# RS2002/PianoBart

Hardware: AMD Instinct MI355X
Metric: Octuple tokens/sec/GPU (seq=1024, 12L/768d) pretrain step; %MFMA peak (higher is better)
Workload: dtype bf16

## Files before the change

### pianobart_amd/csrc/pb_fa_tiles.h

```cpp
#pragma once
#include "pb_common.h"
#include "pb_api_internal.h"

namespace {


constexpr int HD = 64, FT = 256;
constexpr float LOG2E = 1.4426950408889634f;
typedef __attribute__((ext_vector_type(4))) short s16x4;
typedef __attribute__((ext_vector_type(8))) short s16x8;

struct Fa64Args {
    const bf16_t *q, *k, *v, *o, *dout;
    bf16_t *out, *dq, *dk, *dv;
    float* lse; const float* delta; const float* key_mask; const int* kmax;
    int B, H, Sq, Sk;
    long q_sb, q_ss, k_sb, k_ss, v_sb, v_ss, o_sb, o_ss, dq_sb, dq_ss, dk_sb, dk_ss, dv_sb, dv_ss;
    float scale; int causal;
    float* cs_q; float* cs_kv;
    const bf16_t* zeros;
    const int *vl_q_off, *vl_k_off, *vl_q_len, *vl_k_len;
    const int* bh_order;
};

inline Fa64Args fa64_args(const pb_attn_desc& d, bool bwd) {
    Fa64Args a = {};
    a.q = (const bf16_t*)d.q; a.k = (const bf16_t*)d.k; a.v = (const bf16_t*)d.v; a.dout = (const bf16_t*)d.dout;
    if (bwd) a.o = (const bf16_t*)d.o; else a.out = (bf16_t*)d.o;
    a.dq = (bf16_t*)d.dq; a.dk = (bf16_t*)d.dk; a.dv = (bf16_t*)d.dv; a.lse = d.lse; a.delta = d.delta;
    a.key_mask = d.key_mask; a.kmax = d.q_off ? d.k_vis : d.kmax;
    a.B = d.B; a.H = d.H; a.Sq = d.Sq; a.Sk = d.Sk;
    a.q_sb = d.q_sb; a.q_ss = d.q_ss; a.k_sb = d.k_sb; a.k_ss = d.k_ss; a.v_sb = d.v_sb; a.v_ss = d.v_ss; a.o_sb = d.o_sb; a.o_ss = d.o_ss;
    a.dq_sb = d.dq_sb; a.dq_ss = d.dq_ss; a.dk_sb = d.dk_sb; a.dk_ss = d.dk_ss; a.dv_sb = d.dv_sb; a.dv_ss = d.dv_ss;
    a.scale = d.scale; a.causal = d.flags & PB_ATTN_CAUSAL;
    a.zeros = (const bf16_t*)pb_zero_page();
    a.vl_q_off = d.q_off; a.vl_k_off = d.k_off; a.vl_q_len = d.q_len; a.vl_k_len = d.k_len; a.bh_order = d.bh_order;
    return a;
}

__device__ __forceinline__ void varlen_localize(Fa64Args& p, int b) {
    if (!p.vl_q_off) return;
    const long qo = p.vl_q_off[b], ko = p.vl_k_off[b];
    p.Sq = p.vl_q_len[b]; p.Sk = p.vl_k_len[b];
    p.q += qo * p.q_ss - b * p.q_sb; p.k += ko * p.k_ss - b * p.k_sb; p.v += ko * p.v_ss - b * p.v_sb;
    if (p.o) p.o += qo * p.o_ss - b * p.o_sb;
    if (p.out) p.out += qo * p.o_ss - b * p.o_sb;
    if (p.dout) p.dout += qo * p.o_ss - b * p.o_sb;
    if (p.dq) p.dq += qo * p.dq_ss - b * p.dq_sb;
    if (p.dk) p.dk += ko * p.dk_ss - b * p.dk_sb;
    if (p.dv) p.dv += ko * p.dv_ss - b * p.dv_sb;
}

#define MFMA16(a, b, c) __builtin_amdgcn_mfma_f32_16x16x32_bf16((a), (b), (c), 0, 0, 0)

__device__ __forceinline__ int fsw(int row) { return (((row >> 1) & 3) << 1) | ((row >> 3) & 1); }

__device__ __forceinline__ void glds16(const bf16_t* g, char* lds_wave_base) {
    __builtin_amdgcn_global_load_lds((const __attribute__((address_space(1))) void*)g,
                                     (__attribute__((address_space(3))) void*)lds_wave_base, 16, 0, 0);
}
struct StageOff { unsigned off[2]; unsigned chunk[2]; };
__device__ __forceinline__ StageOff stage_off(long ld, int wave, int lane) {
    StageOff o;
#pragma unroll
    for (int n = 0; n < 2; ++n) {
        const int row = (wave * 2 + n) * 8 + (lane >> 3);
        o.chunk[n] = (unsigned)((lane & 7) ^ fsw(row));
        o.off[n] = (unsigned)(row * ld + (o.chunk[n] << 3));
    }
    return o;
}
__device__ __forceinline__ void stage64(const bf16_t* __restrict__ base, long ld, int r0, int nrows, char* lds, int wave, int lane, const StageOff& so,
                                        int cmax = 8, const bf16_t* zeros = nullptr) {
    if (r0 + 64 <= nrows) {
        const bf16_t* tb = base + (long)r0 * ld;
#pragma unroll
        for (int n = 0; n < 2; ++n) glds16((cmax == 8 || (int)so.chunk[n] < cmax) ? tb + so.off[n] : zeros, lds + (wave * 2 + n) * 1024);
    } else {
#pragma unroll
        for (int n = 0; n < 2; ++n) {
            const int inst = wave * 2 + n;
            const int row = inst * 8 + (lane >> 3);
            const int chunk = (lane & 7) ^ fsw(row);
            const int gr = min(r0 + row, nrows - 1);
            glds16((cmax == 8 || chunk < cmax) ? base + (long)gr * ld + chunk * 8 : zeros, lds + inst * 1024);
        }
    }
}
__device__ __forceinline__ bf16x8 frag_row(const char* lds, int row, int ks, int g) {
    return *reinterpret_cast<const bf16x8*>(lds + row * 128 + (((ks * 4 + g) ^ fsw(row)) << 4));
}
__device__ __forceinline__ bf16x8 frag_tr(const char* lds, int c0, int s, int lane) {
    const int lr = lane & 15, g = lane >> 4, qq = lr >> 2, pp = lr & 3;
    const int chunk = (c0 >> 3) + (pp >> 1);
    const int r0 = 32 * s + 4 * g + qq, r1 = r0 + 16;
    const int o0 = r0 * 128 + ((chunk ^ fsw(r0)) << 4) + ((pp & 1) << 3);
    const int o1 = r1 * 128 + ((chunk ^ fsw(r1)) << 4) + ((pp & 1) << 3);
    const s16x4 lo = __builtin_amdgcn_ds_read_tr16_b64_v4i16((__attribute__((address_space(3))) s16x4*)(lds + o0));
    const s16x4 hi = __builtin_amdgcn_ds_read_tr16_b64_v4i16((__attribute__((address_space(3))) s16x4*)(lds + o1));
    const s16x8 v = {lo[0], lo[1], lo[2], lo[3], hi[0], hi[1], hi[2], hi[3]};
    return __builtin_bit_cast(bf16x8, v);
}
__device__ __forceinline__ bf16x8 pack_pair(const f32x4& lo, const f32x4& hi) {
    bf16x8 r = {(bf16_t)lo[0], (bf16_t)lo[1], (bf16_t)lo[2], (bf16_t)lo[3], (bf16_t)hi[0], (bf16_t)hi[1], (bf16_t)hi[2], (bf16_t)hi[3]};
    return r;
}
__device__ __forceinline__ bf16x8 frag_global(const bf16_t* __restrict__ g, long ld, int row, int nvalid, int col) {
    bf16x8 z = {};
    if (row < nvalid) z = *reinterpret_cast<const bf16x8*>(g + (long)row * ld + col);
    return z;
}
__device__ __forceinline__ float grp_max(float v) {
    auto a = __builtin_amdgcn_permlane16_swap(__float_as_uint(v), __float_as_uint(v), false, false);
    v = fmaxf(__uint_as_float(a[0]), __uint_as_float(a[1]));
    auto b = __builtin_amdgcn_permlane32_swap(__float_as_uint(v), __float_as_uint(v), false, false);
    return fmaxf(__uint_as_float(b[0]), __uint_as_float(b[1]));
}
__device__ __forceinline__ float grp_sum(float v) {
    auto a = __builtin_amdgcn_permlane16_swap(__float_as_uint(v), __float_as_uint(v), false, false);
    v = __uint_as_float(a[0]) + __uint_as_float(a[1]);
    auto b = __builtin_amdgcn_permlane32_swap(__float_as_uint(v), __float_as_uint(v), false, false);
    return __uint_as_float(b[0]) + __uint_as_float(b[1]);
}
template <bool V> struct BoolTag { static constexpr bool value = V; };

constexpr int STG = 2 * 8192 + 512;

__device__ __forceinline__ void block_map(int nrb, int H, int B, int& rb, int& h, int& b, const int* order = nullptr) {
    const int L = blockIdx.x, BH = H * B;
    int bh;
    if ((BH & 7) == 0) { const int x = L & 7, slot = L >> 3, j = slot / nrb; bh = j * 8 + x; rb = (slot - j * nrb + j) % nrb; }
    else { bh = L / nrb; rb = (L - bh * nrb + bh) % nrb; }
    if (order) bh = order[bh];
    h = bh % H; b = bh / H;
}

template <int OFF>
__device__ __forceinline__ void ds_tr(s16x4& d, unsigned addr) {
    asm volatile("ds_read_b64_tr_b16 %0, %1 offset:%2" : "=v"(d) : "v"(addr), "i"(OFF));
}
__device__ __forceinline__ unsigned tr_lane_off64(int c0, int lane) {
    const int lr = lane & 15, g = lane >> 4, qq = lr >> 2, pp = lr & 3;
    const int r0 = 4 * g + qq, chunk = (c0 >> 3) + (pp >> 1);
    return (unsigned)(r0 * 128 + ((chunk ^ fsw(r0)) << 4) + ((pp & 1) << 3));
}
__device__ __forceinline__ void ds_tr_block(s16x4 (&d)[2][2], unsigned addr) {
    ds_tr<0>(d[0][0], addr); ds_tr<2048>(d[0][1], addr); ds_tr<4096>(d[1][0], addr); ds_tr<6144>(d[1][1], addr);
}
__device__ __forceinline__ bf16x8 tr_join(s16x4 lo, s16x4 hi) {
    const s16x8 v = {lo[0], lo[1], lo[2], lo[3], hi[0], hi[1], hi[2], hi[3]};
    return __builtin_bit_cast(bf16x8, v);
}
#define TRW4(X) "+v"(X[0][0]), "+v"(X[0][1]), "+v"(X[1][0]), "+v"(X[1][1])
__device__ __forceinline__ void tr_wait4(s16x4 (&t)[4][2][2]) {
    asm volatile("s_waitcnt lgkmcnt(0)" : TRW4(t[0]), TRW4(t[1]), TRW4(t[2]), TRW4(t[3]));
}
__device__ __forceinline__ void tr_wait8(s16x4 (&t)[4][2][2], s16x4 (&u)[4][2][2]) {
    asm volatile("s_waitcnt lgkmcnt(0)" : TRW4(t[0]), TRW4(t[1]), TRW4(t[2]), TRW4(t[3]), TRW4(u[0]), TRW4(u[1]), TRW4(u[2]), TRW4(u[3]));
}
#undef TRW4
__device__ __forceinline__ unsigned lds_u32(const void* p) { return (unsigned)(uintptr_t)(__attribute__((address_space(3))) const char*)p; }

template <int N> __device__ __forceinline__ void wait_vm() { asm volatile("s_waitcnt vmcnt(%0)" :: "i"(N) : "memory"); }

template <int NB> struct FaCfg {
    static constexpr int NS = NB == 1 ? 3 : 2;
    static constexpr int STB = 2 * NB * 8192;
    static constexpr int PCS = 4 * NB;
    static constexpr int KT = NB == 1 ? 2 : 1;
};

__device__ __forceinline__ bf16x8 scale_frag(bf16x8 v, float c) {
    bf16x8 r;
#pragma unroll
    for (int e = 0; e < 8; ++e) r[e] = (bf16_t)((float)v[e] * c);
    return r;
}

}
```

### pianobart_amd/csrc/pb_flash64.hip

```cpp
#include "pb_common.h"
#include "pb_fa_tiles.h"

namespace {


constexpr float LAZY_THR = 8.0f;
template <int HD>
__global__ __launch_bounds__(FT) void fa64_fwd_kernel(const Fa64Args pin) {
    constexpr int NB = (HD + 63) / 64, KS = HD / 32, DT = HD / 16, HDT = HD;
    using C = FaCfg<NB>;
    extern __shared__ __attribute__((aligned(16))) char smem[];
    const int t = threadIdx.x, lane = t & 63, lr = lane & 15, g = lane >> 4;
    const int wave = __builtin_amdgcn_readfirstlane(t >> 6);
    int rb, h, b;
    block_map((pin.Sq + 127) / 128, pin.H, pin.B, rb, h, b, pin.bh_order);
    if (pin.causal) rb = (pin.Sq + 127) / 128 - 1 - rb;
    const int q0 = rb * 128;
    Fa64Args p = pin;
    varlen_localize(p, b);
    const int lse_ld = pin.Sq;
    if (q0 >= p.Sq) return;
    const bf16_t* Q = p.q + b * p.q_sb + h * HDT;
    const bf16_t* K = p.k + b * p.k_sb + h * HDT;
    const bf16_t* V = p.v + b * p.v_sb + h * HDT;
    const float c = p.scale * LOG2E;
    const int kvis_end = p.kmax ? min(p.Sk, p.kmax[b]) : p.Sk;
    const int kend = p.causal ? min(kvis_end, q0 + 128) : kvis_end;
    const int nt = (kend + 63) / 64;
    float* ldsBias = reinterpret_cast<float*>(smem + C::NS * C::STB);
    unsigned* ldsFlag = reinterpret_cast<unsigned*>(ldsBias + ((p.Sk + 63) / 64) * 64);
    for (int tile = wave; tile < nt; tile += 4) {
        const int key = tile * 64 + lane;
        const bool vis = key < (pin.vl_q_off ? kvis_end : p.Sk) && (!p.key_mask || p.key_mask[(long)b * p.Sk + key] != 0.f);
        ldsBias[key] = vis ? 0.f : -INFINITY;
        const bool allvis = __builtin_amdgcn_ballot_w64(vis) == ~0ull;
        if (lane == 0) ldsFlag[tile] = allvis ? 0u : 1u;
    }
    int myq[2];
    bf16x8 qf[2][KS];
#pragma unroll
    for (int qt = 0; qt < 2; ++qt) {
        myq[qt] = q0 + wave * 32 + qt * 16 + lr;
#pragma unroll
        for (int ks = 0; ks < KS; ++ks) qf[qt][ks] = scale_frag(frag_global(Q, p.q_ss, myq[qt], p.Sq, ks * 32 + g * 8), c);
    }
#pragma unroll
    for (int ks = 0; ks < KS; ++ks) asm volatile("" : "+v"(qf[0][ks]), "+v"(qf[1][ks]));
    f32x4 oacc[2][DT];
#pragma unroll
    for (int qt = 0; qt < 2; ++qt)
#pragma unroll
        for (int i = 0; i < DT; ++i) oacc[qt][i] = f32x4{0.f, 0.f, 0.f, 0.f};
    float m[2] = {-INFINITY, -INFINITY};
    f32x4 cinit[2] = {f32x4{0.f, 0.f, 0.f, 0.f}, f32x4{0.f, 0.f, 0.f, 0.f}};
    f32x4 lacc[2] = {f32x4{0.f, 0.f, 0.f, 0.f}, f32x4{0.f, 0.f, 0.f, 0.f}};
    const bf16_t one = (bf16_t)1.0f;
    const bf16x8 ones = {one, one, one, one, one, one, one, one};
    unsigned voff[4];
#pragma unroll
    for (int dt = 0; dt < 4; ++dt) voff[dt] = lds_u32(smem) + NB * 8192 + tr_lane_off64(dt * 16, lane);
    const StageOff so_k = stage_off(p.k_ss, wave, lane), so_v = stage_off(p.v_ss, wave, lane);
    auto stage = [&](int it, int sidx) {
        char* st = smem + sidx * C::STB;
#pragma unroll
        for (int nb = 0; nb < NB; ++nb) {
            stage64(K + nb * 64, p.k_ss, it * 64, p.Sk, st + nb * 8192, wave, lane, so_k, min(8, (HD - nb * 64) / 8), p.zeros);
            stage64(V + nb * 64, p.v_ss, it * 64, p.Sk, st + (NB + nb) * 8192, wave, lane, so_v, min(8, (HD - nb * 64) / 8), p.zeros);
        }
    };
    if (nt > 0) stage(0, 0);
    if (C::NS == 3 && nt > 1) { stage(1, 1); wait_vm<C::PCS>(); } else { wait_vm<0>(); }
    __builtin_amdgcn_s_waitcnt(0xc07f);
    __builtin_amdgcn_s_barrier();
    int sidx = 0;
    for (int it = 0; it < nt; ++it) {
        const char* st = smem + sidx * C::STB;
        const int nidx = sidx == 0 ? C::NS - 1 : sidx - 1;
        if (it + C::NS - 1 < nt) stage(it + C::NS - 1, nidx);
        const float* ldsB = ldsBias + it * 64;
        const int k0 = it * 64;
        const bool diag = p.causal && (k0 + 63 > q0 + wave * 32);
        const bool masked = diag || __builtin_amdgcn_readfirstlane(ldsFlag[it]) != 0u;
        f32x4 s[2][4];
#pragma unroll
        for (int kt = 0; kt < 4; ++kt) {
#pragma unroll
            for (int qt = 0; qt < 2; ++qt) s[qt][kt] = cinit[qt];
#pragma unroll
            for (int nb = 0; nb < NB; ++nb) {
#pragma unroll
                for (int k2 = 0; k2 < 2; ++k2)
                    if (2 * nb + k2 < KS) {
                        const bf16x8 kk = frag_row(st + nb * 8192, kt * 16 + lr, k2, g);
#pragma unroll
                        for (int qt = 0; qt < 2; ++qt) s[qt][kt] = MFMA16(kk, qf[qt][2 * nb + k2], s[qt][kt]);
                    }
            }
        }
        s16x4 tv[4][2][2];
#pragma unroll
        for (int dt = 0; dt < 4; ++dt) if (dt < DT) ds_tr_block(tv[dt], voff[dt] + (unsigned)(sidx * C::STB));
        bf16x8 pf[2][2];
        auto finish_row = [&](int qt) {
            pf[qt][0] = pack_pair(s[qt][0], s[qt][1]);
            pf[qt][1] = pack_pair(s[qt][2], s[qt][3]);
            lacc[qt] = MFMA16(ones, pf[qt][1], MFMA16(ones, pf[qt][0], lacc[qt]));
        };
        float resc[2] = {1.f, 1.f};
        auto exact_tile = [&](auto tag) {
            constexpr bool MASKED = decltype(tag)::value;
            asm volatile("; exact softmax path" ::: "memory");
#pragma unroll
            for (int qt = 0; qt < 2; ++qt) {
                const float mold = m[qt] == -INFINITY ? 0.f : m[qt];
                float mx = -INFINITY;
#pragma unroll
                for (int kt = 0; kt < 4; ++kt) {
                    f32x4 bias = {0.f, 0.f, 0.f, 0.f};
                    if constexpr (MASKED) bias = *reinterpret_cast<const f32x4*>(ldsB + kt * 16 + g * 4);
#pragma unroll
                    for (int r = 0; r < 4; ++r) {
                        float x = s[qt][kt][r] + mold;
                        if constexpr (MASKED) {
                            x += bias[r];
                            if (diag && (k0 + kt * 16 + g * 4 + r) > myq[qt]) x = -INFINITY;
                        }
                        s[qt][kt][r] = x;
                        mx = fmaxf(mx, x);
                    }
                }
                mx = grp_max(mx);
                const float mnew = fmaxf(m[qt], mx);
                const float muse = mnew == -INFINITY ? 0.f : mnew;
                const float alpha = __builtin_amdgcn_exp2f(m[qt] - muse);
#pragma unroll
                for (int kt = 0; kt < 4; ++kt)
#pragma unroll
                    for (int r = 0; r < 4; ++r) s[qt][kt][r] = __builtin_amdgcn_exp2f(s[qt][kt][r] - muse);
                lacc[qt] *= alpha;
                m[qt] = mnew;
                cinit[qt] = f32x4{-muse, -muse, -muse, -muse};
                resc[qt] = alpha;
                finish_row(qt);
            }
        };
        bool exact = masked;
        if (masked) {
            exact_tile(BoolTag<true>{});
        } else {
            float t0 = m[0] == -INFINITY ? INFINITY : -INFINITY, t1 = m[1] == -INFINITY ? INFINITY : -INFINITY;
#pragma unroll
            for (int kt = 0; kt < 4; ++kt)
#pragma unroll
                for (int r = 0; r < 4; ++r) { t0 = fmaxf(t0, s[0][kt][r]); t1 = fmaxf(t1, s[1][kt][r]); }
            if (__builtin_amdgcn_ballot_w64(fmaxf(t0, t1) > LAZY_THR) == 0ull) {
#pragma unroll
                for (int qt = 0; qt < 2; ++qt) {
#pragma unroll
                    for (int kt = 0; kt < 4; ++kt)
#pragma unroll
                        for (int r = 0; r < 4; ++r) s[qt][kt][r] = __builtin_amdgcn_exp2f(s[qt][kt][r]);
                    finish_row(qt);
                }
            } else {
                exact = true;
                exact_tile(BoolTag<false>{});
            }
        }
        if (exact) {
#pragma unroll
            for (int qt = 0; qt < 2; ++qt)
#pragma unroll
                for (int i = 0; i < DT; ++i) oacc[qt][i] *= resc[qt];
        }
#pragma unroll
        for (int nb = 0; nb < NB; ++nb) {
            if (nb > 0) {
#pragma unroll
                for (int dt = 0; dt < 4; ++dt) if (nb * 4 + dt < DT) ds_tr_block(tv[dt], voff[dt] + (unsigned)(sidx * C::STB + nb * 8192));
            }
            tr_wait4(tv);
#pragma unroll
            for (int dt = 0; dt < 4; ++dt) if (nb * 4 + dt < DT) {
                const bf16x8 v0 = tr_join(tv[dt][0][0], tv[dt][0][1]), v1 = tr_join(tv[dt][1][0], tv[dt][1][1]);
#pragma unroll
                for (int qt = 0; qt < 2; ++qt) oacc[qt][nb * 4 + dt] = MFMA16(v1, pf[qt][1], MFMA16(v0, pf[qt][0], oacc[qt][nb * 4 + dt]));
            }
        }
        if (C::NS == 3 && it + 2 < nt) { wait_vm<C::PCS>(); } else { wait_vm<0>(); }
        __builtin_amdgcn_s_barrier();
        sidx = sidx == C::NS - 1 ? 0 : sidx + 1;
    }
    if constexpr (HD == 64) {
        typedef __attribute__((ext_vector_type(2))) unsigned u32x2;
        typedef __attribute__((ext_vector_type(4))) unsigned u32x4;
        const unsigned obase = lds_u32(smem) + (unsigned)(wave * 4096);
#pragma unroll
        for (int qt = 0; qt < 2; ++qt) {
            const float lq = lacc[qt][0];
            const float inv = lq > 0.f ? 1.0f / lq : 0.f;
#pragma unroll
            for (int dt = 0; dt < DT; ++dt) {
                const bf16x4 r = {(bf16_t)(oacc[qt][dt][0] * inv), (bf16_t)(oacc[qt][dt][1] * inv), (bf16_t)(oacc[qt][dt][2] * inv), (bf16_t)(oacc[qt][dt][3] * inv)};
                *reinterpret_cast<__attribute__((address_space(3))) u32x2*>(obase + (unsigned)(qt * 2048 + lr * 128 + ((((dt * 2 + (g >> 1)) ^ (lr & 7)) << 4) | ((g & 1) << 3)))) =
                    __builtin_bit_cast(u32x2, r);
            }
            if (myq[qt] < p.Sq && g == 0) p.lse[((long)b * p.H + h) * lse_ld + myq[qt]] = lq > 0.f ? (m[qt] + log2f(lq)) / LOG2E : INFINITY;
        }
        const int orow = lane >> 3, ochunk = lane & 7;
#pragma unroll
        for (int qt = 0; qt < 2; ++qt)
#pragma unroll
            for (int hh = 0; hh < 2; ++hh) {
                const int r = hh * 8 + orow, q = q0 + wave * 32 + qt * 16 + r;
                const u32x4 v = *reinterpret_cast<const __attribute__((address_space(3))) u32x4*>(obase + (unsigned)(qt * 2048 + r * 128 + ((ochunk ^ (r & 7)) << 4)));
                if (q < p.Sq) *reinterpret_cast<u32x4*>(p.out + b * p.o_sb + (long)q * p.o_ss + h * HDT + ochunk * 8) = v;
            }
    } else {
#pragma unroll
    for (int qt = 0; qt < 2; ++qt) {
        if (myq[qt] < p.Sq) {
            const float lq = lacc[qt][0];
            const float inv = lq > 0.f ? 1.0f / lq : 0.f;
            bf16_t* O = p.out + b * p.o_sb + (long)myq[qt] * p.o_ss + h * HDT;
#pragma unroll
            for (int dt = 0; dt < DT; ++dt) {
                bf16x4 r = {(bf16_t)(oacc[qt][dt][0] * inv), (bf16_t)(oacc[qt][dt][1] * inv), (bf16_t)(oacc[qt][dt][2] * inv), (bf16_t)(oacc[qt][dt][3] * inv)};
                *reinterpret_cast<bf16x4*>(O + dt * 16 + g * 4) = r;
            }
            if (g == 0) p.lse[((long)b * p.H + h) * lse_ld + myq[qt]] = lq > 0.f ? (m[qt] + log2f(lq)) / LOG2E : INFINITY;
        }
    }
    }
}

template <int HD>
__global__ __launch_bounds__(FT) void fa64_bwd_dkv_kernel(const Fa64Args pin) {
    constexpr int NB = (HD + 63) / 64, KS = HD / 32, DT = HD / 16, HDT = HD;
    using C = FaCfg<NB>;
    constexpr int KT = C::KT, BK_ = 64 * KT;
    extern __shared__ __attribute__((aligned(16))) char smem[];
    const int t = threadIdx.x, lane = t & 63, lr = lane & 15, g = lane >> 4;
    const int wave = __builtin_amdgcn_readfirstlane(t >> 6);
    int rb, h, b;
    block_map((pin.Sk + BK_ - 1) / BK_, pin.H, pin.B, rb, h, b, pin.bh_order);
    const int k0 = rb * BK_;
    Fa64Args p = pin;
    varlen_localize(p, b);
    const int lse_ld = pin.Sq;
    if (k0 >= p.Sk) {
        if (p.cs_kv && t < 2 * HDT) {
            const int nkb0 = (pin.Sk + BK_ - 1) / BK_, dm = p.H * HDT;
            float* row = p.cs_kv + (long)(b * nkb0 + rb) * 2 * dm + h * HDT;
            row[t < HDT ? t : dm + t - HDT] = 0.f;
        }
        return;
    }
    const bf16_t* Q = p.q + b * p.q_sb + h * HDT;
    const bf16_t* K = p.k + b * p.k_sb + h * HDT;
    const bf16_t* V = p.v + b * p.v_sb + h * HDT;
    const bf16_t* DO = p.dout + b * p.o_sb + h * HDT;
    const float c = p.scale * LOG2E;
    const int it0 = p.causal ? k0 / 64 : 0;
    const int nt = (p.kmax && k0 >= p.kmax[b]) ? 0 : (p.Sq + 63) / 64;
    const int sqp = ((p.Sq + 63) / 64) * 64;
    float* ldsNL = reinterpret_cast<float*>(smem + C::NS * C::STB);
    float* ldsND = ldsNL + sqp;
    {
        const long li0 = ((long)b * p.H + h) * lse_ld;
        for (int qb = it0 * 64; qb < nt * 64; qb += 4 * FT) {
            float tl[4], td[4];
#pragma unroll
            for (int i = 0; i < 4; ++i) {
                const int q = qb + t + i * FT;
                tl[i] = q < p.Sq ? p.lse[li0 + q] : INFINITY;
                td[i] = q < p.Sq ? p.delta[li0 + q] : 0.f;
            }
#pragma unroll
            for (int i = 0; i < 4; ++i) {
                const int q = qb + t + i * FT;
                if (q < nt * 64) { ldsNL[q] = tl[i] == INFINITY ? -INFINITY : -tl[i] * LOG2E; ldsND[q] = -td[i]; }
            }
        }
    }
    int mykey[KT];
    bf16x8 kf[KT][KS], vf[KT][KS];
#pragma unroll
    for (int kt = 0; kt < KT; ++kt) {
        mykey[kt] = k0 + wave * (16 * KT) + kt * 16 + lr;
#pragma unroll
        for (int ks = 0; ks < KS; ++ks) {
            kf[kt][ks] = scale_frag(frag_global(K, p.k_ss, mykey[kt], p.Sk, ks * 32 + g * 8), c);
            vf[kt][ks] = frag_global(V, p.v_ss, mykey[kt], p.Sk, ks * 32 + g * 8);
        }
    }
#pragma unroll
    for (int kt = 0; kt < KT; ++kt)
#pragma unroll
        for (int ks = 0; ks < KS; ++ks) asm volatile("" : "+v"(kf[kt][ks]), "+v"(vf[kt][ks]));
    f32x4 dk[KT][DT], dv[KT][DT];
#pragma unroll
    for (int kt = 0; kt < KT; ++kt)
#pragma unroll
        for (int i = 0; i < DT; ++i) { dk[kt][i] = f32x4{0.f, 0.f, 0.f, 0.f}; dv[kt][i] = f32x4{0.f, 0.f, 0.f, 0.f}; }
    unsigned qoff[4], ooff[4];
#pragma unroll
    for (int dt = 0; dt < 4; ++dt) { qoff[dt] = lds_u32(smem) + tr_lane_off64(dt * 16, lane); ooff[dt] = qoff[dt] + NB * 8192; }
    const StageOff so_q = stage_off(p.q_ss, wave, lane), so_o = stage_off(p.o_ss, wave, lane);
    auto stage = [&](int it, int sidx) {
        char* st = smem + sidx * C::STB;
#pragma unroll
        for (int nb = 0; nb < NB; ++nb) {
            stage64(Q + nb * 64, p.q_ss, it * 64, p.Sq, st + nb * 8192, wave, lane, so_q, min(8, (HD - nb * 64) / 8), p.zeros);
            stage64(DO + nb * 64, p.o_ss, it * 64, p.Sq, st + (NB + nb) * 8192, wave, lane, so_o, min(8, (HD - nb * 64) / 8), p.zeros);
        }
    };
    if (it0 < nt) stage(it0, 0);
    if (C::NS == 3 && it0 + 1 < nt) { stage(it0 + 1, 1); wait_vm<C::PCS>(); } else { wait_vm<0>(); }
    __builtin_amdgcn_s_waitcnt(0xc07f);
    __builtin_amdgcn_s_barrier();
    int sidx = 0;
    for (int it = it0; it < nt; ++it) {
        const char* st = smem + sidx * C::STB;
        const int nidx = sidx == 0 ? C::NS - 1 : sidx - 1;
        if (it + C::NS - 1 < nt) stage(it + C::NS - 1, nidx);
        const int q0 = it * 64;
        const bool diag = p.causal && (k0 + wave * (16 * KT) + 16 * KT - 1 > q0);
        bf16x8 pf[KT][2], df[KT][2];
#pragma unroll
        for (int half = 0; half < 2; ++half) {
            f32x4 sv[KT][2], dp[KT][2];
#pragma unroll
            for (int qq = 0; qq < 2; ++qq) {
                const int qt = half * 2 + qq;
                const f32x4 nl = *reinterpret_cast<const f32x4*>(ldsNL + q0 + qt * 16 + g * 4);
                const f32x4 nd = *reinterpret_cast<const f32x4*>(ldsND + q0 + qt * 16 + g * 4);
#pragma unroll
                for (int kt = 0; kt < KT; ++kt) { sv[kt][qq] = nl; dp[kt][qq] = nd; }
#pragma unroll
                for (int nb = 0; nb < NB; ++nb) {
                    const char* ldsQ = st + nb * 8192; const char* ldsO = st + (NB + nb) * 8192;
#pragma unroll
                    for (int k2 = 0; k2 < 2; ++k2)
                        if (2 * nb + k2 < KS) {
                            const bf16x8 qa = frag_row(ldsQ, qt * 16 + lr, k2, g), oa = frag_row(ldsO, qt * 16 + lr, k2, g);
#pragma unroll
                            for (int kt = 0; kt < KT; ++kt) {
                                sv[kt][qq] = MFMA16(qa, kf[kt][2 * nb + k2], sv[kt][qq]);
                                dp[kt][qq] = MFMA16(oa, vf[kt][2 * nb + k2], dp[kt][qq]);
                            }
                        }
                }
            }
            if (diag) {
#pragma unroll
                for (int kt = 0; kt < KT; ++kt)
#pragma unroll
                    for (int qq = 0; qq < 2; ++qq)
#pragma unroll
                        for (int r = 0; r < 4; ++r) {
                            const int q = q0 + (half * 2 + qq) * 16 + g * 4 + r;
                            const float pr = mykey[kt] <= q ? __builtin_amdgcn_exp2f(sv[kt][qq][r]) : 0.f;
                            sv[kt][qq][r] = pr; dp[kt][qq][r] *= pr;
                        }
            } else {
#pragma unroll
                for (int kt = 0; kt < KT; ++kt)
#pragma unroll
                    for (int qq = 0; qq < 2; ++qq)
#pragma unroll
                        for (int r = 0; r < 4; ++r) {
                            const float pr = __builtin_amdgcn_exp2f(sv[kt][qq][r]);
                            sv[kt][qq][r] = pr; dp[kt][qq][r] *= pr;
                        }
            }
#pragma unroll
            for (int kt = 0; kt < KT; ++kt) { pf[kt][half] = pack_pair(sv[kt][0], sv[kt][1]); df[kt][half] = pack_pair(dp[kt][0], dp[kt][1]); }
        }
#pragma unroll
        for (int nb = 0; nb < NB; ++nb)
#pragma unroll
        for (int si = 0; si < 2; ++si) {
            s16x4 to[4][2], tq[4][2];
#pragma unroll
            for (int dt = 0; dt < 4; ++dt) if (nb * 4 + dt < DT) {
                const unsigned ao = ooff[dt] + (unsigned)(sidx * C::STB + nb * 8192), aq = qoff[dt] + (unsigned)(sidx * C::STB + nb * 8192);
                if (si == 0) { ds_tr<0>(to[dt][0], ao); ds_tr<2048>(to[dt][1], ao); ds_tr<0>(tq[dt][0], aq); ds_tr<2048>(tq[dt][1], aq); }
                else { ds_tr<4096>(to[dt][0], ao); ds_tr<6144>(to[dt][1], ao); ds_tr<4096>(tq[dt][0], aq); ds_tr<6144>(tq[dt][1], aq); }
            }
            asm volatile("s_waitcnt lgkmcnt(0)" : "+v"(to[0][0]), "+v"(to[0][1]), "+v"(to[1][0]), "+v"(to[1][1]), "+v"(to[2][0]), "+v"(to[2][1]), "+v"(to[3][0]), "+v"(to[3][1]),
                                                  "+v"(tq[0][0]), "+v"(tq[0][1]), "+v"(tq[1][0]), "+v"(tq[1][1]), "+v"(tq[2][0]), "+v"(tq[2][1]), "+v"(tq[3][0]), "+v"(tq[3][1]));
#pragma unroll
            for (int dt = 0; dt < 4; ++dt) if (nb * 4 + dt < DT) {
                const bf16x8 ot = tr_join(to[dt][0], to[dt][1]), qtf = tr_join(tq[dt][0], tq[dt][1]);
#pragma unroll
                for (int kt = 0; kt < KT; ++kt) {
                    dv[kt][nb * 4 + dt] = MFMA16(ot, pf[kt][si], dv[kt][nb * 4 + dt]);
                    dk[kt][nb * 4 + dt] = MFMA16(qtf, df[kt][si], dk[kt][nb * 4 + dt]);
                }
            }
        }
        if (C::NS == 3 && it + 2 < nt) { wait_vm<C::PCS>(); } else { wait_vm<0>(); }
        __builtin_amdgcn_s_barrier();
        sidx = sidx == C::NS - 1 ? 0 : sidx + 1;
    }
    f32x4 csk[DT], csv[DT];
#pragma unroll
    for (int dt = 0; dt < DT; ++dt) { csk[dt] = f32x4{0.f, 0.f, 0.f, 0.f}; csv[dt] = f32x4{0.f, 0.f, 0.f, 0.f}; }
    if constexpr (HD == 64) {
        typedef __attribute__((ext_vector_type(2))) unsigned u32x2;
        typedef __attribute__((ext_vector_type(4))) unsigned u32x4;
        const unsigned obase = lds_u32(smem) + 4096u + (unsigned)(wave * (KT * 4096));
#pragma unroll
        for (int kt = 0; kt < KT; ++kt) {
            const int key = k0 + wave * (16 * KT) + kt * 16 + lr;
            const bool kvis = pin.vl_q_off ? key < (p.kmax ? p.kmax[b] : p.Sk)
                                           : (!p.key_mask || p.key_mask[(long)b * p.Sk + (key < p.Sk ? key : 0)] != 0.f);
#pragma unroll
            for (int dt = 0; dt < DT; ++dt) {
                f32x4 vk = dk[kt][dt] * p.scale, vv = dv[kt][dt];
                if (!kvis) { vk = f32x4{0.f, 0.f, 0.f, 0.f}; vv = f32x4{0.f, 0.f, 0.f, 0.f}; }
                const bf16x4 rk = {(bf16_t)vk[0], (bf16_t)vk[1], (bf16_t)vk[2], (bf16_t)vk[3]}, rv = {(bf16_t)vv[0], (bf16_t)vv[1], (bf16_t)vv[2], (bf16_t)vv[3]};
                const unsigned slot = (unsigned)(lr * 128 + ((((dt * 2 + (g >> 1)) ^ (lr & 7)) << 4) | ((g & 1) << 3)));
                *reinterpret_cast<__attribute__((address_space(3))) u32x2*>(obase + (unsigned)(kt * 4096) + slot) = __builtin_bit_cast(u32x2, rk);
                *reinterpret_cast<__attribute__((address_space(3))) u32x2*>(obase + (unsigned)(kt * 4096 + 2048) + slot) = __builtin_bit_cast(u32x2, rv);
                if (key < p.Sk) { csk[dt] += vk; csv[dt] += vv; }
            }
        }
        const int orow = lane >> 3, ochunk = lane & 7;
#pragma unroll
        for (int kt = 0; kt < KT; ++kt)
#pragma unroll
            for (int hh = 0; hh < 2; ++hh) {
                const int r = hh * 8 + orow, key = k0 + wave * (16 * KT) + kt * 16 + r;
                const unsigned slot = (unsigned)(r * 128 + ((ochunk ^ (r & 7)) << 4));
                const u32x4 vk = *reinterpret_cast<const __attribute__((address_space(3))) u32x4*>(obase + (unsigned)(kt * 4096) + slot);
                const u32x4 vv = *reinterpret_cast<const __attribute__((address_space(3))) u32x4*>(obase + (unsigned)(kt * 4096 + 2048) + slot);
                if (key < p.Sk) {
                    *reinterpret_cast<u32x4*>(p.dk + b * p.dk_sb + (long)key * p.dk_ss + h * HDT + ochunk * 8) = vk;
                    *reinterpret_cast<u32x4*>(p.dv + b * p.dv_sb + (long)key * p.dv_ss + h * HDT + ochunk * 8) = vv;
                }
            }
    } else {
#pragma unroll
    for (int kt = 0; kt < KT; ++kt) {
        const int key = k0 + wave * (16 * KT) + kt * 16 + lr;
        const bool kvis = pin.vl_q_off ? key < (p.kmax ? p.kmax[b] : p.Sk)
                                       : (!p.key_mask || p.key_mask[(long)b * p.Sk + (key < p.Sk ? key : 0)] != 0.f);
        bf16_t* DK = p.dk + b * p.dk_sb + (long)key * p.dk_ss + h * HDT + g * 4;
        bf16_t* DV = p.dv + b * p.dv_sb + (long)key * p.dv_ss + h * HDT + g * 4;
#pragma unroll
        for (int dt = 0; dt < DT; ++dt) {
            f32x4 vk = dk[kt][dt] * p.scale, vv = dv[kt][dt];
            if (!kvis) { vk = f32x4{0.f, 0.f, 0.f, 0.f}; vv = f32x4{0.f, 0.f, 0.f, 0.f}; }
            if (key < p.Sk) {
                bf16x4 rk = {(bf16_t)vk[0], (bf16_t)vk[1], (bf16_t)vk[2], (bf16_t)vk[3]}, rv = {(bf16_t)vv[0], (bf16_t)vv[1], (bf16_t)vv[2], (bf16_t)vv[3]};
                *reinterpret_cast<bf16x4*>(DK + dt * 16) = rk;
                *reinterpret_cast<bf16x4*>(DV + dt * 16) = rv;
                csk[dt] += vk; csv[dt] += vv;
            }
        }
    }
    }
    if (p.cs_kv) {
        const int nkb = (pin.Sk + BK_ - 1) / BK_, d_model = p.H * HDT;
        float* red = reinterpret_cast<float*>(smem);
#pragma unroll
        for (int dt = 0; dt < DT; ++dt) {
#pragma unroll
            for (int e = 0; e < 4; ++e) {
                float v = csk[dt][e], u = csv[dt][e];
                v += PB_DPP_F(v, 0x140); u += PB_DPP_F(u, 0x140);
                v += PB_DPP_F(v, 0x141); u += PB_DPP_F(u, 0x141);
                v += PB_DPP_F(v, 0x4e); u += PB_DPP_F(u, 0x4e);
                v += PB_DPP_F(v, 0xb1); u += PB_DPP_F(u, 0xb1);
                csk[dt][e] = v; csv[dt][e] = u;
            }
            if (lr == 0) {
                *reinterpret_cast<f32x4*>(red + wave * 2 * HDT + dt * 16 + g * 4) = csk[dt];
                *reinterpret_cast<f32x4*>(red + wave * 2 * HDT + HDT + dt * 16 + g * 4) = csv[dt];
            }
        }
        __syncthreads();
        if (t < 2 * HDT) {
            float* row = p.cs_kv + (long)(b * nkb + rb) * 2 * d_model + h * HDT;
            const float v = red[t] + red[2 * HDT + t] + red[4 * HDT + t] + red[6 * HDT + t];
            row[t < HDT ? t : d_model + t - HDT] = v;
        }
    }
}

template <int HD>
__global__ __launch_bounds__(FT) void fa64_bwd_dq_kernel(const Fa64Args pin) {
    constexpr int NB = (HD + 63) / 64, KS = HD / 32, DT = HD / 16, HDT = HD;
    using C = FaCfg<NB>;
    extern __shared__ __attribute__((aligned(16))) char smem[];
    const int t = threadIdx.x, lane = t & 63, lr = lane & 15, g = lane >> 4;
    const int wave = __builtin_amdgcn_readfirstlane(t >> 6);
    int rb, h, b;
// ... 270 lines not shown
```

Baseline: 622,200.

## Software-pipeline HD=64 flash forward with next-tile QK overlapped into softmax/PV

Adds a dedicated HD=64 forward path that splits K and V staging, prefetching K three tiles ahead and V two ahead, and computes the next tile's QK^T scores while the current tile's exp/pack/PV work runs. A hand-scheduled lazy-rescale branch interleaves MFMAs with exp2 and pack operations using sched_barrier. Waits now also drain LDS (lgkmcnt), and a waves_per_eu hint is added. The aim is to hide MFMA latency and global-load latency, at the cost of higher register pressure and considerably more complex code.

Result: no change. 624,000 (median of 6 runs) (+0.3%).

```diff
diff --git a/pianobart_amd/csrc/pb_fa_tiles.h b/pianobart_amd/csrc/pb_fa_tiles.h
--- a/pianobart_amd/csrc/pb_fa_tiles.h
+++ b/pianobart_amd/csrc/pb_fa_tiles.h
@@ -162,6 +162,7 @@
 __device__ __forceinline__ unsigned lds_u32(const void* p) { return (unsigned)(uintptr_t)(__attribute__((address_space(3))) const char*)p; }
 
 template <int N> __device__ __forceinline__ void wait_vm() { asm volatile("s_waitcnt vmcnt(%0)" :: "i"(N) : "memory"); }
+template <int N> __device__ __forceinline__ void wait_vm_lds() { asm volatile("s_waitcnt vmcnt(%0) lgkmcnt(0)" :: "i"(N) : "memory"); }
 
 template <int NB> struct FaCfg {
     static constexpr int NS = NB == 1 ? 3 : 2;
diff --git a/pianobart_amd/csrc/pb_flash64.hip b/pianobart_amd/csrc/pb_flash64.hip
--- a/pianobart_amd/csrc/pb_flash64.hip
+++ b/pianobart_amd/csrc/pb_flash64.hip
@@ -6,7 +6,7 @@
 
 constexpr float LAZY_THR = 8.0f;
 template <int HD>
-__global__ __launch_bounds__(FT) void fa64_fwd_kernel(const Fa64Args pin) {
+__global__ __launch_bounds__(FT) __attribute__((amdgpu_waves_per_eu(HD == 64 ? 2 : 1))) void fa64_fwd_kernel(const Fa64Args pin) {
     constexpr int NB = (HD + 63) / 64, KS = HD / 32, DT = HD / 16, HDT = HD;
     using C = FaCfg<NB>;
     extern __shared__ __attribute__((aligned(16))) char smem[];
@@ -60,6 +60,229 @@
 #pragma unroll
     for (int dt = 0; dt < 4; ++dt) voff[dt] = lds_u32(smem) + NB * 8192 + tr_lane_off64(dt * 16, lane);
     const StageOff so_k = stage_off(p.k_ss, wave, lane), so_v = stage_off(p.v_ss, wave, lane);
+    if constexpr (HD == 64) {
+    constexpr unsigned STB = C::STB;
+    auto stage_k = [&](int j, unsigned off, int ln) { stage64(K, p.k_ss, j * 64, p.Sk, smem + off, wave, ln, so_k, 8, p.zeros); };
+    auto stage_v = [&](int j, unsigned off, int ln) { stage64(V, p.v_ss, j * 64, p.Sk, smem + off + 8192, wave, ln, so_v, 8, p.zeros); };
+    auto s_chain = [&](f32x4 (&s)[2][4], const bf16x8 ka, const bf16x8 kb, int kt) __attribute__((always_inline)) {
+#pragma unroll
+        for (int qt = 0; qt < 2; ++qt) s[qt][kt] = MFMA16(ka, qf[qt][0], cinit[qt]);
+#pragma unroll
+        for (int qt = 0; qt < 2; ++qt) s[qt][kt] = MFMA16(kb, qf[qt][1], s[qt][kt]);
+    };
+    if (nt > 0) stage_k(0, 0, lane);
+    if (nt > 1) stage_k(1, STB, lane);
+    if (nt > 0) stage_v(0, 0, lane);
+    if (nt > 2) stage_k(2, 2 * STB, lane);
+    if (nt > 1) stage_v(1, STB, lane);
+    if (nt > 2) wait_vm<4>(); else if (nt > 1) wait_vm<2>(); else wait_vm<0>();
+    __builtin_amdgcn_s_waitcnt(0xc07f);
+    __builtin_amdgcn_s_barrier();
+    f32x4 sA[2][4], sB[2][4];
+    if (nt > 0) {
+#pragma unroll
+        for (int kt = 0; kt < 4; ++kt) s_chain(sA, frag_row(smem, kt * 16 + lr, 0, g), frag_row(smem, kt * 16 + lr, 1, g), kt);
+    }
+    wait_vm_lds<4>();
+    __builtin_amdgcn_s_barrier();
+    auto body = [&](auto next_tag, const int it, f32x4 (&sc)[2][4], f32x4 (&sn)[2][4], const unsigned o0, const unsigned o1, const unsigned o2) __attribute__((always_inline)) {
+        constexpr bool have_next = decltype(next_tag)::value;
+        int ln_s = lane;
+        asm volatile("" : "+v"(ln_s));
+        if (it + 3 < nt) stage_k(it + 3, o0, ln_s);
+        if (it + 2 < nt) stage_v(it + 2, o2, ln_s);
+        const float* ldsB = ldsBias + it * 64;
+        const int k0 = it * 64;
+        const bool diag = p.causal && (k0 + 63 > q0 + wave * 32);
+        const bool masked = diag || __builtin_amdgcn_readfirstlane(ldsFlag[it]) != 0u;
+        const char* kn = smem + o1;
+        s16x4 tv[4][2][2];
+        auto v_request = [&]() __attribute__((always_inline)) {
+#pragma unroll
+            for (int dt = 0; dt < 4; ++dt) ds_tr_block(tv[dt], voff[dt] + o0);
+        };
+        bf16x8 pf[2][2];
+        auto exp_tile = [&](int qt, int kt) __attribute__((always_inline)) {
+#pragma unroll
+            for (int r = 0; r < 4; ++r) sc[qt][kt][r] = __builtin_amdgcn_exp2f(sc[qt][kt][r]);
+        };
+        auto pack_row = [&](int qt) __attribute__((always_inline)) {
+            pf[qt][0] = pack_pair(sc[qt][0], sc[qt][1]);
+            pf[qt][1] = pack_pair(sc[qt][2], sc[qt][3]);
+        };
+        auto sum_row = [&](int qt) __attribute__((always_inline)) {
+            lacc[qt] = MFMA16(ones, pf[qt][1], MFMA16(ones, pf[qt][0], lacc[qt]));
+        };
+        auto pv_row = [&](int qt) __attribute__((always_inline)) {
+#pragma unroll
+            for (int dt = 0; dt < 4; ++dt) {
+                const bf16x8 v0 = tr_join(tv[dt][0][0], tv[dt][0][1]), v1 = tr_join(tv[dt][1][0], tv[dt][1][1]);
+                oacc[qt][dt] = MFMA16(v1, pf[qt][1], MFMA16(v0, pf[qt][0], oacc[qt][dt]));
+            }
+        };
+        auto above_thr = [&]() __attribute__((always_inline)) {
+            float t0 = m[0] == -INFINITY ? INFINITY : -INFINITY, t1 = m[1] == -INFINITY ? INFINITY : -INFINITY;
+#pragma unroll
+            for (int kt = 0; kt < 4; ++kt)
+#pragma unroll
+                for (int r = 0; r < 4; ++r) { t0 = fmaxf(t0, sc[0][kt][r]); t1 = fmaxf(t1, sc[1][kt][r]); }
+            return __builtin_amdgcn_ballot_w64(fmaxf(t0, t1) > LAZY_THR) != 0ull;
+        };
+        float resc[2] = {1.f, 1.f};
+        auto exact_tile = [&](auto tag) __attribute__((always_inline)) {
+            constexpr bool MASKED = decltype(tag)::value;
+            int ln = lane;
+            asm volatile("; exact softmax path" : "+v"(ln) :: "memory");
+            const int lr_x = ln & 15, g_x = ln >> 4;
+#pragma unroll
+            for (int qt = 0; qt < 2; ++qt) {
+                const float mold = m[qt] == -INFINITY ? 0.f : m[qt];
+                const int qlim = diag ? q0 + wave * 32 + qt * 16 + lr_x : 0x7fffffff;
+                float mx = -INFINITY;
+#pragma unroll
+                for (int kt = 0; kt < 4; ++kt) {
+                    f32x4 bias = {0.f, 0.f, 0.f, 0.f};
+                    if constexpr (MASKED) bias = *reinterpret_cast<const f32x4*>(ldsB + kt * 16 + g_x * 4);
+#pragma unroll
+                    for (int r = 0; r < 4; ++r) {
+                        float x = sc[qt][kt][r] + mold;
+                        if constexpr (MASKED) {
+                            x += bias[r];
+                            if ((k0 + kt * 16 + g_x * 4 + r) > qlim) x = -INFINITY;
+                        }
+                        sc[qt][kt][r] = x;
+                        mx = fmaxf(mx, x);
+                    }
+                }
+                mx = grp_max(mx);
+                const float mnew = fmaxf(m[qt], mx);
+                const float muse = mnew == -INFINITY ? 0.f : mnew;
+                const float alpha = __builtin_amdgcn_exp2f(m[qt] - muse);
+#pragma unroll
+                for (int kt = 0; kt < 4; ++kt)
+#pragma unroll
+                    for (int r = 0; r < 4; ++r) sc[qt][kt][r] = __builtin_amdgcn_exp2f(sc[qt][kt][r] - muse);
+                lacc[qt] *= alpha;
+                m[qt] = mnew;
+                cinit[qt] = f32x4{-muse, -muse, -muse, -muse};
+                resc[qt] = alpha;
+                pack_row(qt);
+                sum_row(qt);
+            }
+        };
+        bf16x8 kf[4][2];
+        auto k_read = [&](int kt) __attribute__((always_inline)) { kf[kt][0] = frag_row(kn, kt * 16 + lr, 0, g); kf[kt][1] = frag_row(kn, kt * 16 + lr, 1, g); };
+                auto next_chain = [&](int kt) __attribute__((always_inline)) { if constexpr (have_next) s_chain(sn, kf[kt][0], kf[kt][1], kt); };
+        bool lazy = false;
+        if (!masked && it > 0) {
+            lazy = !above_thr();
+            if (lazy) {
+                if constexpr (have_next) {
+                    typedef __attribute__((ext_vector_type(2))) bf16_t bf16x2;
+                    typedef __attribute__((ext_vector_type(4))) unsigned u32x4;
+                    unsigned pw[2][8];
+                    auto ex = [&](int qt, int i) __attribute__((always_inline)) { sc[qt][i >> 2][i & 3] = __builtin_amdgcn_exp2f(sc[qt][i >> 2][i & 3]); };
+                    auto pk = [&](int qt, int i) __attribute__((always_inline)) {
+                        const bf16x2 t = {(bf16_t)sc[qt][i >> 1][(i & 1) * 2], (bf16_t)sc[qt][i >> 1][(i & 1) * 2 + 1]};
+                        pw[qt][i] = __builtin_bit_cast(unsigned, t);
+                    };
+                    auto join = [&](int qt) __attribute__((always_inline)) {
+                        pf[qt][0] = __builtin_bit_cast(bf16x8, u32x4{pw[qt][0], pw[qt][1], pw[qt][2], pw[qt][3]});
+                        pf[qt][1] = __builtin_bit_cast(bf16x8, u32x4{pw[qt][4], pw[qt][5], pw[qt][6], pw[qt][7]});
+                    };
+                    auto step = []() __attribute__((always_inline)) { __builtin_amdgcn_sched_barrier(0); };
+                    k_read(0); k_read(1);
+                    ex(0, 0); ex(0, 1); ex(0, 2); ex(0, 3);
+                    step();
+#pragma unroll
+                    for (int kt = 0; kt < 4; ++kt) {
+#pragma unroll
+                        for (int s = 0; s < 4; ++s) {
+                            const int qt = s & 1, n = kt * 4 + s;
+                            sn[qt][kt] = s < 2 ? MFMA16(kf[kt][0], qf[qt][0], cinit[qt]) : MFMA16(kf[kt][1], qf[qt][1], sn[qt][kt]);
+                            if (n < 12) ex(0, 4 + n); else { pk(0, 2 * (n - 12)); pk(0, 2 * (n - 12) + 1); }
+                            if (s == 1 && kt < 2) k_read(kt + 2);
+                            step();
+                        }
+                    }
+                    join(0);
+                    v_request();
+#pragma unroll
+                    for (int i = 0; i < 8; ++i) ex(1, i);
+#pragma unroll
+                    for (int i = 0; i < 4; ++i) pk(1, i);
+                    tr_wait4(tv);
+                    step();
+                    bf16x8 va[4], vb[4];
+#pragma unroll
+                    for (int dt = 0; dt < 4; ++dt) { va[dt] = tr_join(tv[dt][0][0], tv[dt][0][1]); vb[dt] = tr_join(tv[dt][1][0], tv[dt][1][1]); }
+                    auto pv_pinned = [&](int qt, bool fill) __attribute__((always_inline)) {
+                        int n = 0;
+                        auto behind = [&]() __attribute__((always_inline)) {
+                            if (fill) {
+                                if (n < 8) ex(1, 8 + n);
+                                if (n == 4 || n == 5) pk(1, n);
+                                if (n == 8) { pk(1, 6); pk(1, 7); }
+                            }
+                            ++n;
+                            step();
+                        };
+                        lacc[qt] = MFMA16(ones, pf[qt][0], lacc[qt]); behind();
+                        oacc[qt][0] = MFMA16(va[0], pf[qt][0], oacc[qt][0]); behind();
+                        lacc[qt] = MFMA16(ones, pf[qt][1], lacc[qt]); behind();
+                        oacc[qt][0] = MFMA16(vb[0], pf[qt][1], oacc[qt][0]); behind();
+                        oacc[qt][1] = MFMA16(va[1], pf[qt][0], oacc[qt][1]); behind();
+                        oacc[qt][2] = MFMA16(va[2], pf[qt][0], oacc[qt][2]); behind();
+                        oacc[qt][1] = MFMA16(vb[1], pf[qt][1], oacc[qt][1]); behind();
+                        oacc[qt][2] = MFMA16(vb[2], pf[qt][1], oacc[qt][2]); behind();
+                        oacc[qt][3] = MFMA16(va[3], pf[qt][0], oacc[qt][3]); behind();
+                        oacc[qt][3] = MFMA16(vb[3], pf[qt][1], oacc[qt][3]); behind();
+                        if (fill) join(1);
+                    };
+                    pv_pinned(0, true);
+                    pv_pinned(1, false);
+                } else {
+#pragma unroll
+                    for (int qt = 0; qt < 2; ++qt) {
+#pragma unroll
+                        for (int kt = 0; kt < 4; ++kt) exp_tile(qt, kt);
+                        pack_row(qt);
+                    }
+                    v_request();
+                    tr_wait4(tv);
+                    sum_row(0); pv_row(0); sum_row(1); pv_row(1);
+                }
+            }
+        }
+        if (!lazy) {
+            if (masked) exact_tile(BoolTag<true>{}); else exact_tile(BoolTag<false>{});
+#pragma unroll
+            for (int kt = 0; kt < 4; ++kt) { if constexpr (have_next) k_read(kt); next_chain(kt); }
+            v_request();
+#pragma unroll
+            for (int qt = 0; qt < 2; ++qt)
+#pragma unroll
+                for (int i = 0; i < DT; ++i) oacc[qt][i] *= resc[qt];
+            tr_wait4(tv);
+            pv_row(0); pv_row(1);
+        }
+        if (it + 3 < nt) wait_vm_lds<4>(); else if (it + 2 < nt) wait_vm_lds<2>(); else wait_vm_lds<0>();
+        __builtin_amdgcn_s_barrier();
+    };
+    unsigned o0 = 0, o1 = STB, o2 = 2 * STB;
+    int it = 0;
+    for (; it + 2 < nt; it += 2) {
+        body(BoolTag<true>{}, it, sA, sB, o0, o1, o2);
+        body(BoolTag<true>{}, it + 1, sB, sA, o1, o2, o0);
+        const unsigned o = o2; o2 = o1; o1 = o0; o0 = o;
+    }
+    if (it + 1 < nt) {
+        body(BoolTag<true>{}, it, sA, sB, o0, o1, o2);
+        body(BoolTag<false>{}, it + 1, sB, sA, o1, o2, o0);
+    } else if (it < nt) {
+        body(BoolTag<false>{}, it, sA, sB, o0, o1, o2);
+    }
+    } else {
     auto stage = [&](int it, int sidx) {
         char* st = smem + sidx * C::STB;
 #pragma unroll
@@ -191,10 +414,15 @@
         __builtin_amdgcn_s_barrier();
         sidx = sidx == C::NS - 1 ? 0 : sidx + 1;
     }
+    }
     if constexpr (HD == 64) {
         typedef __attribute__((ext_vector_type(2))) unsigned u32x2;
         typedef __attribute__((ext_vector_type(4))) unsigned u32x4;
         const unsigned obase = lds_u32(smem) + (unsigned)(wave * 4096);
+        int lane_e = lane;
+        asm volatile("" : "+v"(lane_e));
+        const int lane = lane_e, lr = lane & 15, g = lane >> 4;
+        const int myq[2] = {q0 + wave * 32 + lr, q0 + wave * 32 + 16 + lr};
 #pragma unroll
         for (int qt = 0; qt < 2; ++qt) {
             const float lq = lacc[qt][0];
```
